# yxgeee/OpenIBL

Hardware: NVIDIA H100
Metric: images_per_sec_extraction (higher is better)
Workload: dtype f32 (bf16x3 split on wgmma, fp32 accumulate)

## Files before the change

include/iblb200.h:

```cpp
#ifndef IBLB200_H_
#define IBLB200_H_

#include <stddef.h>
#include <stdint.h>

#ifdef __cplusplus
extern "C" {
#endif

#define IBLB200_ABI_VERSION 1

typedef enum ibl_status {
  IBL_OK = 0,
  IBL_ERR_BAD_ARG = 1,
  IBL_ERR_NOT_READY = 2,
  IBL_ERR_CUDA = 3,
  IBL_ERR_NO_DEVICE = 4,
  IBL_ERR_OOM = 5,
  IBL_ERR_UNSUPPORTED = 6
} ibl_status;

typedef struct ibl_engine ibl_engine;

#define IBL_OUT_VLAD 0x1u
// ... 99 lines not shown
                   int m, int k_in, int k_out, float* out_dist, int64_t* out_idx, void* stream);
int ibl_l2dist_topk_host(ibl_engine* e, const float* q_host, int m, const float* db_host, int n,
                         int d, int k, float* out_dist_host, int64_t* out_idx_host, void* stream);

int ibl_knn_rowmax(ibl_engine* e, const float* X, int N, int d, int row0, int n_rows, int w, int64_t* out_idx,
                   float* out_dist, float* out_rowmax, void* stream);
int ibl_rerank_topk(ibl_engine* e, const float* X, int N, int m, int d, const int64_t* nbr_idx, const float* nbr_dist,
                    int w, const float* rowmax, int k1, int k2, float lambda_value, const int64_t* orig_idx, int k_orig,
                    int k, float* out_dist, int64_t* out_idx, void* stream);
int ibl_rerank_dense(ibl_engine* e, const float* qg, const float* qq, const float* gg, int m, int n, int k1, int k2,
                     double lambda_value, float* out_final, void* stream);

int ibl_gemm_nt(ibl_engine* e, const float* A, int m, const float* B, int n, int k, float alpha, float* C, int mode,
                void* stream);

int ibl_debug_dist_flagged(ibl_engine* e, int* count, void* stream);
int ibl_debug_dist_path(ibl_engine* e, int* path);
int ibl_debug_knn_flagged(ibl_engine* e, int* count, void* stream);
int ibl_debug_rerank_workspace_bytes(ibl_engine* e, uint64_t* bytes);
int ibl_selftest_tc(ibl_engine* e, float* max_rel_err);

int ibl_debug_conv3x3(ibl_engine* e, const float* x_nhwc, int N, int H, int W, int cin,
                      const float* w_oihw, const float* bias, int cout, int relu, int pool, int mode,
                      int bn_override, float* y_nhwc, void* stream);

int ibl_debug_gemm_tn(ibl_engine* e, const float* A, const float* B, float* C, void* stream);
int ibl_debug_umma_strided(ibl_engine* e, const void* A, int rows, const void* B, int s0, int group_rows,
                           int base_mode, float* D, void* stream);
int ibl_debug_umma_halo_view(ibl_engine* e, const void* A, int rows, const void* B, int s0, int group_rows,
                             int half_rows, float* D, void* stream);
int ibl_debug_conv1_fused(ibl_engine* e, const float* x, int N, int H, int W, void* y_hi, void* y_lo, void* stream);
int ibl_debug_time_layer(ibl_engine* e, int layer, const float* x, int N, int H, int W, int bn_override,
                         int reps, float* ms_out);

#ifdef __cplusplus
}
#endif
#endif
```

openibl_b200/_cabi.py:

```python
from __future__ import annotations

import ctypes
import os
from ctypes import POINTER, Structure, c_char, c_char_p, c_double, c_float, c_int, c_int64, c_size_t, c_uint, c_uint64, c_void_p

_HERE = os.path.dirname(os.path.abspath(__file__))
LIB_PATH = os.path.join(_HERE, "lib", "libiblb200.so")

IBL_OK = 0
STATUS_NAMES = {0: "IBL_OK", 1: "IBL_ERR_BAD_ARG", 2: "IBL_ERR_NOT_READY", 3: "IBL_ERR_CUDA",
                4: "IBL_ERR_NO_DEVICE", 5: "IBL_ERR_OOM", 6: "IBL_ERR_UNSUPPORTED"}
OUT_VLAD, OUT_PCA, OUT_POOL = 0x1, 0x2, 0x4
CONV_SIMT_FP32, CONV_TC_BF16X3 = 0, 1

_P = c_void_p


class JpegInfo(Structure):
    _fields_ = [("width", c_int), ("height", c_int), ("components", c_int), ("h_samp", c_int), ("v_samp", c_int),
                ("restart_interval", c_int), ("intervals", c_int), ("mcus", c_int), ("entropy_bytes", c_uint64),
                ("reason", c_char * 120)]


class ColorJitterParams(Structure):
# ... 27 lines not shown
    "ibl_l2_normalize_rows": (c_int, [_P, _P, c_int, c_int, _P, _P]),
    "ibl_extract": (c_int, [_P, _P, c_int, c_int, c_int, c_uint, _P, _P, _P]),
    "ibl_extract_host": (c_int, [_P, _P, c_int, c_int, c_int, c_uint, _P, _P, _P]),
    "ibl_extract_host_submit": (c_int, [_P, c_int, _P, c_int, c_int, c_int, c_uint, _P, _P, _P]),
    "ibl_extract_host_wait": (c_int, [_P, c_int]),
    "ibl_preprocess_u8": (c_int, [_P, _P, c_int, c_int, c_int, _P, _P, _P, _P]),
    "ibl_resize_bilinear_u8": (c_int, [_P, _P, c_int, c_int, c_int, c_int, c_int, _P, _P, c_int, _P, _P, c_int, _P, _P]),
    "ibl_extract_host_u8": (c_int, [_P, _P, c_int, c_int, c_int, _P, _P, c_uint, _P, _P, _P]),
    "ibl_jpeg_parse": (c_int, [c_char_p, c_size_t, POINTER(JpegInfo)]),
    "ibl_jpeg_decode_u8": (c_int, [_P, _P, _P, c_int, _P, _P, _P, _P, _P]),
    "ibl_color_jitter_u8": (c_int, [_P, _P, _P, _P, _P, POINTER(ColorJitterParams), c_int, _P]),
    "ibl_l2dist_dense": (c_int, [_P, _P, c_int, _P, c_int, c_int, _P, _P]),
    "ibl_l2dist_self": (c_int, [_P, _P, c_int, c_int, _P, _P]),
    "ibl_l2dist_topk": (c_int, [_P, _P, c_int, _P, c_int, c_int, c_int, c_int, c_int64, _P, _P, _P]),
    "ibl_topk_rows": (c_int, [_P, _P, c_int, c_int, c_int, _P, _P, _P]),
    "ibl_argsort_rows": (c_int, [_P, _P, c_int, c_int, _P, _P]),
    "ibl_topk_merge": (c_int, [_P, _P, _P, c_int, c_int, c_int, c_int, _P, _P, _P]),
    "ibl_l2dist_topk_host": (c_int, [_P, _P, c_int, _P, c_int, c_int, c_int, _P, _P, _P]),
    "ibl_knn_rowmax": (c_int, [_P, _P, c_int, c_int, c_int, c_int, c_int, _P, _P, _P, _P]),
    "ibl_rerank_topk": (c_int, [_P, _P, c_int, c_int, c_int, _P, _P, c_int, _P, c_int, c_int, c_float, _P, c_int,
                                c_int, _P, _P, _P]),
    "ibl_rerank_dense": (c_int, [_P, _P, _P, _P, c_int, c_int, c_int, c_int, c_double, _P, _P]),
    "ibl_debug_rerank_workspace_bytes": (c_int, [_P, POINTER(c_uint64)]),
    "ibl_debug_knn_flagged": (c_int, [_P, POINTER(c_int), _P]),
    "ibl_gemm_nt": (c_int, [_P, _P, c_int, _P, c_int, c_int, c_float, _P, c_int, _P]),
    "ibl_debug_dist_flagged": (c_int, [_P, POINTER(c_int), _P]),
    "ibl_debug_dist_path": (c_int, [_P, POINTER(c_int)]),
    "ibl_selftest_tc": (c_int, [_P, POINTER(c_float)]),
    "ibl_debug_gemm_tn": (c_int, [_P, _P, _P, _P, _P]),
    "ibl_debug_umma_strided": (c_int, [_P, _P, c_int, _P, c_int, c_int, c_int, _P, _P]),
    "ibl_debug_umma_halo_view": (c_int, [_P, _P, c_int, _P, c_int, c_int, c_int, _P, _P]),
    "ibl_debug_conv1_fused": (c_int, [_P, _P, c_int, c_int, c_int, _P, _P, _P]),
    "ibl_debug_time_layer": (c_int, [_P, c_int, _P, c_int, c_int, c_int, c_int, c_int, POINTER(c_float)]),
    "ibl_debug_conv3x3": (c_int, [_P, _P, c_int, c_int, c_int, c_int, _P, _P, c_int, c_int, c_int, c_int,
                                  c_int, _P, _P]),
}

_lib = None


class IblError(RuntimeError):
    def __init__(self, status: int, where: str, detail: str):
        self.status = status
        super().__init__(f"{where}: {STATUS_NAMES.get(status, status)}: {detail}")


def load(build_if_missing: bool = True) -> ctypes.CDLL:
    global _lib
    if _lib is not None:
        return _lib
    if not os.path.exists(LIB_PATH):
        if not build_if_missing:
            raise ImportError(f"{LIB_PATH} is missing; run `python -m openibl_b200.build`")
        from . import build as _build
        _build.build()
    lib = ctypes.CDLL(LIB_PATH)
    for name, (res, args) in SIGNATURES.items():
        fn = getattr(lib, name)
        fn.restype = res
        fn.argtypes = args
    _lib = lib
    return lib


def jpeg_parse(data: bytes) -> dict:
    lib = load()
# ... 15 lines not shown
```

openibl_b200/csrc/common.cuh:

```cuda
#pragma once
#include <cuda_runtime.h>
#include <cuda_bf16.h>
#include <stdint.h>
#include <stdio.h>
#include <atomic>
#include <string>

#include "../../include/iblb200.h"

namespace ibl {

void set_last_error(const std::string& s);

#define IBL_CUDA_OK(expr)                                                          \
  do {                                                                             \
    cudaError_t _e = (expr);                                                       \
    if (_e != cudaSuccess) {                                                       \
      ::ibl::set_last_error(std::string(#expr) + ": " + cudaGetErrorString(_e) +   \
                            " (" __FILE__ ":" + std::to_string(__LINE__) + ")");   \
      return IBL_ERR_CUDA;                                                         \
    }                                                                              \
  } while (0)

#define IBL_RET(expr)                 \
// ... 44 lines not shown
  int cin, cout;
  bool relu;
  bool pool;
};

struct ConvParams {
  float* w_tck = nullptr;
  float* bias = nullptr;
  __nv_bfloat16* w_hi = nullptr;
  __nv_bfloat16* w_lo = nullptr;
  int cin_pad = 0;
};

int launch_repack_weights(const float* w_oihw, int cout, int cin, ConvParams& p, cudaStream_t s);
int launch_conv3x3_simt(const float* x_nhwc, const ConvParams& p, int N, int H, int W, int cin,
                        int cout, bool relu, float* y_nhwc, cudaStream_t s);
int launch_conv1_1(const float* x_nchw, const ConvParams& p, int N, int H, int W, float* y_nhwc, cudaStream_t s);
int launch_maxpool2x2(const float* x, int N, int H, int W, int C, float* y, cudaStream_t s);
int launch_nhwc_to_nchw(const float* x, int N, int S, int C, float* y, cudaStream_t s);
int launch_u8_hwc_to_nchw_norm(const uint8_t* x, int N, int H, int W, const float* mean, const float* stdv, float* y,
                               cudaStream_t s);
int launch_global_maxpool_nhwc(const float* x, int N, int S, int C, float* y, cudaStream_t s);
int launch_planes_to_f32(const __nv_bfloat16* hi, const __nv_bfloat16* lo, size_t n, float* y,
                         cudaStream_t s);
int launch_f32_to_planes(const float* x, size_t n, __nv_bfloat16* hi, __nv_bfloat16* lo,
                         cudaStream_t s);

struct TcConvPlan;
int tc_driver_init();
int launch_conv3x3_tc(const __nv_bfloat16* x_hi, const __nv_bfloat16* x_lo, const ConvParams& p,
                      int N, int H, int W, int cin, int cout, bool relu, bool pool,
                      __nv_bfloat16* y_hi, __nv_bfloat16* y_lo, float* y_f32, cudaStream_t s,
                      float* ssq = nullptr, int* ssq_parts = nullptr);
int launch_conv1_fused_tc(const float* x_nchw, const float* w1_oihw, const float* bias1, const ConvParams& p2, int N, int H,
                          int W, __nv_bfloat16* y_hi, __nv_bfloat16* y_lo, cudaStream_t s);
int launch_maxpool2x2_planes(const __nv_bfloat16* hi, const __nv_bfloat16* lo, int N, int H, int W,
                             int C, __nv_bfloat16* yhi, __nv_bfloat16* ylo, cudaStream_t s);
int tc_selftest(float* max_rel_err, cudaStream_t s);
int launch_argsort_rows(const float* dist, long long ld, int m, int n, long long* idx, unsigned long long* scratch,
                        cudaStream_t s, uint64_t* launches);
int launch_resize_bilinear_u8(const uint8_t* x, int N, int Hin, int Win, int Hout, int Wout, const int* bounds_h,
                              const int* kk_h, int ksize_h, const int* bounds_v, const int* kk_v, int ksize_v,
                              uint8_t* tmp, uint8_t* out, cudaStream_t s, uint64_t* launches);
struct JpegWs;
void jpeg_ws_destroy(JpegWs* ws);
int jpeg_decode_u8(JpegWs** ws, const uint8_t* const* files, const size_t* lens, int N, uint8_t* out_u8,
                   const uint64_t* out_offsets, int* status, int* err_dev, cudaStream_t s, uint64_t* launches);
struct JitterWs;
void jitter_ws_destroy(JitterWs* ws);
int color_jitter_u8(JitterWs** ws, uint8_t* buf, const uint64_t* out_offsets, const int* H, const int* W,
                    const ibl_color_jitter_params* params, int N, cudaStream_t s, uint64_t* launches);
int launch_repack_weights_dgrad(const float* w_tck, int cout, int cin, __nv_bfloat16* w_hi, __nv_bfloat16* w_lo,
                                cudaStream_t s);
int launch_relu_mask_planes(const float* g, const float* y, size_t n, bool relu, __nv_bfloat16* hi, __nv_bfloat16* lo,
                            cudaStream_t s);
int launch_maxpool2x2_bwd(const float* x, const float* gy, int N, int H, int W, int C, float* gx, cudaStream_t s);
int wgrad_tc_splits(int N, int H, int W, int cin, int cout);
int launch_conv_wgrad_tc(const __nv_bfloat16* g_hi, const __nv_bfloat16* g_lo, const __nv_bfloat16* x_hi,
                         const __nv_bfloat16* x_lo, int N, int H, int W, int cin, int cout, float* part, int splits,
                         float* bpart, float* dw_oihw, float* db, cudaStream_t s);
int launch_conv1_1_wgrad(const float* x_nchw, const __nv_bfloat16* g_hi, const __nv_bfloat16* g_lo, int N, int H, int W,
                         float* part, float* dw_oihw, float* db, cudaStream_t s);
int launch_conv1_1_tc(const float* x_nchw, const float* w_oihw, const float* bias, int N, int H, int W,
                      __nv_bfloat16* y_hi, __nv_bfloat16* y_lo, cudaStream_t s);
int debug_gmma_strided(const void* A, int rows, const void* B, int s0, int group_rows, int half_rows, int base_mode,
                       float* D, cudaStream_t s);
// ... 88 lines not shown
```

openibl_b200/csrc/engine.cu:

```cuda
#include <stdlib.h>

#include <mutex>
#include <new>
#include <vector>

#include "common.cuh"

namespace ibl {

static thread_local std::string g_last_error;
void set_last_error(const std::string& s) { g_last_error = s; }
void tc_set_bn_override(int bn);

static const ConvLayer kVgg16[13] = {
    {3, 64, true, false},    {64, 64, true, true},
    {64, 128, true, false},  {128, 128, true, true},
    {128, 256, true, false}, {256, 256, true, false}, {256, 256, true, true},
    {256, 512, true, false}, {512, 512, true, false}, {512, 512, true, true},
    {512, 512, true, false}, {512, 512, true, false}, {512, 512, false, false}
};

struct DevBuf {
  void* p = nullptr;
  size_t cap = 0;
// ... 1241 lines not shown
  IBL_RET(e->act[1].ensure((in_e > out_e ? in_e : out_e) * 4));
  cudaEvent_t e0, e1;
  IBL_CUDA_OK(cudaEventCreate(&e0));
  IBL_CUDA_OK(cudaEventCreate(&e1));
  __nv_bfloat16* ih = e->act[0].as<__nv_bfloat16>();
  __nv_bfloat16* oh_ = e->act[1].as<__nv_bfloat16>();
  int rc = IBL_OK;
  if (layer > 0) rc = launch_f32_to_planes(x, in_e, ih, ih + in_e, nullptr);
  tc_set_bn_override(bn_override);
  for (int r = -1; r < reps && rc == IBL_OK; ++r) {
    if (r == 0) cudaEventRecord(e0, nullptr);
    if (fused1)
      rc = launch_conv1_fused_tc(x, e->w0_oihw, e->conv[0].bias, e->conv[1], N, H, W, oh_, oh_ + out_e, nullptr);
    else if (layer == 0)
      rc = launch_conv1_1_tc(x, e->w0_oihw, e->conv[0].bias, N, H, W, oh_, oh_ + out_e, nullptr);
    else
      rc = launch_conv3x3_tc(ih, ih + in_e, e->conv[layer], N, H, W, L.cin, L.cout, L.relu, L.pool,
                             layer == 12 ? nullptr : oh_, layer == 12 ? nullptr : oh_ + out_e,
                             layer == 12 ? e->act[1].as<float>() : nullptr, nullptr);
  }
  tc_set_bn_override(0);
  cudaEventRecord(e1, nullptr);
  cudaError_t ce = cudaEventSynchronize(e1);
  float ms = 0.f;
  cudaEventElapsedTime(&ms, e0, e1);
  cudaEventDestroy(e0);
  cudaEventDestroy(e1);
  if (rc == IBL_OK && ce != cudaSuccess) { set_last_error(cudaGetErrorString(ce)); return IBL_ERR_CUDA; }
  *ms_out = ms / reps;
  e->launches += reps + 1;
  return rc;
}

}
```

openibl_b200/csrc/tc_common.cuh:

```cuda
#pragma once
#include <cuda.h>
#include <cuda_runtime.h>
#include <stdint.h>

#include "wgmma.cuh"

namespace ibl {
namespace tc {

__device__ __forceinline__ uint32_t smem_u32(const void* p) {
  return static_cast<uint32_t>(__cvta_generic_to_shared(p));
}

__device__ __forceinline__ uint32_t warp_uniform(uint32_t v) { return __reduce_or_sync(0xffffffffu, v); }

__device__ __forceinline__ bool elect_one() {
  uint32_t pred;
  asm volatile(
      "{\n\t"
      ".reg .pred p;\n\t"
      "elect.sync _|p, 0xffffffff;\n\t"
      "selp.u32 %0, 1, 0, p;\n\t"
      "}"
      : "=r"(pred));
// ... 113 lines not shown
__device__ __forceinline__ void tma_load_2d_mc_a(uint32_t dst, const CUtensorMap* m, uint32_t bar_addr, int c0, int c1,
                                                 uint16_t mask) {
  asm volatile(
      "cp.async.bulk.tensor.2d.shared::cluster.global.mbarrier::complete_tx::bytes.multicast::cluster"
      " [%0], [%1, {%4, %5}], [%2], %3;" ::"r"(dst),
      "l"(reinterpret_cast<uint64_t>(m)), "r"(bar_addr), "h"(mask), "r"(c0), "r"(c1)
      : "memory");
}
__device__ __forceinline__ void tma_load_3d_mc_a(uint32_t dst, const CUtensorMap* m, uint32_t bar_addr, int c0, int c1,
                                                 int c2, uint16_t mask) {
  asm volatile(
      "cp.async.bulk.tensor.3d.shared::cluster.global.mbarrier::complete_tx::bytes.multicast::cluster"
      " [%0], [%1, {%4, %5, %6}], [%2], %3;" ::"r"(dst),
      "l"(reinterpret_cast<uint64_t>(m)), "r"(bar_addr), "h"(mask), "r"(c0), "r"(c1), "r"(c2)
      : "memory");
}
__device__ __forceinline__ void cluster_sync_all() {
  asm volatile("barrier.cluster.arrive.release.aligned;" ::: "memory");
  asm volatile("barrier.cluster.wait.acquire.aligned;" ::: "memory");
}
__device__ __forceinline__ uint32_t cluster_ctarank() {
  uint32_t r;
  asm volatile("mov.u32 %0, %%cluster_ctarank;" : "=r"(r));
  return r;
}
__device__ __forceinline__ uint32_t mapa_u32(uint32_t addr, uint32_t rank) {
  uint32_t r;
  asm volatile("mapa.shared::cluster.u32 %0, %1, %2;" : "=r"(r) : "r"(addr), "r"(rank));
  return r;
}
__device__ __forceinline__ void mbar_arrive_remote(uint32_t cluster_addr) {
  asm volatile("mbarrier.arrive.release.cluster.shared::cluster.b64 _, [%0];" ::"r"(cluster_addr) : "memory");
}

__device__ __forceinline__ void tma_prefetch_3d(const CUtensorMap* m, int c0, int c1, int c2) {
  asm volatile("cp.async.bulk.prefetch.tensor.3d.L2.global [%0, {%1, %2, %3}];" ::"l"(
                   reinterpret_cast<uint64_t>(m)),
               "r"(c0), "r"(c1), "r"(c2)
               : "memory");
}

__device__ __forceinline__ uint64_t gmma_desc_kmajor_sw128(uint32_t smem_addr) {
  uint64_t d = 0;
  d |= (uint64_t)((smem_addr >> 4) & 0x3fffu);
  d |= (uint64_t)1 << 16;
  d |= (uint64_t)(1024u >> 4) << 32;
  d |= (uint64_t)1 << 62;
  return d;
}
__device__ __forceinline__ uint64_t gmma_desc_kmajor_sw64(uint32_t smem_addr) {
  uint64_t d = 0;
  d |= (uint64_t)((smem_addr >> 4) & 0x3fffu);
  d |= (uint64_t)1 << 16;
  d |= (uint64_t)(512u >> 4) << 32;
  d |= (uint64_t)2 << 62;
  return d;
}
__device__ __forceinline__ uint64_t gmma_desc_mnmajor_sw128(uint32_t smem_addr, uint32_t lbo_bytes) {
  uint64_t d = 0;
  d |= (uint64_t)((smem_addr >> 4) & 0x3fffu);
  d |= (uint64_t)((lbo_bytes >> 4) & 0x3fffu) << 16;
  d |= (uint64_t)(1024u >> 4) << 32;
  d |= (uint64_t)1 << 62;
  return d;
}

// ... 65 lines not shown
```

openibl_b200/csrc/tc_conv.cu:

```cuda
#include "common.cuh"
#include "tc_common.cuh"

namespace ibl {

using namespace tc;

namespace tc {
EncodeTiledFn get_encode_tiled() {
  static const EncodeTiledFn fn = []() -> EncodeTiledFn {
    void* p = nullptr;
    cudaDriverEntryPointQueryResult qres;
    if (cudaGetDriverEntryPoint("cuTensorMapEncodeTiled", &p, cudaEnableDefault, &qres) ==
            cudaSuccess &&
        qres == cudaDriverEntryPointSuccess)
      return reinterpret_cast<EncodeTiledFn>(p);
    return nullptr;
  }();
  return fn;
}

int make_tmap(CUtensorMap* out, CUtensorMapDataType dt, int rank, const void* base,
              const uint64_t* dims, const uint64_t* strides_bytes, const uint32_t* box, int swizzle_bytes) {
  EncodeTiledFn enc = get_encode_tiled();
  if (!enc) {
    set_last_error("cuTensorMapEncodeTiled is not available (no CUDA driver?)");
    return IBL_ERR_NO_DEVICE;
  }
  cuuint64_t gdim[5];
  cuuint64_t gstr[5];
  cuuint32_t bx[5], es[5];
  for (int i = 0; i < rank; ++i) {
    gdim[i] = dims[i];
    bx[i] = box[i];
    es[i] = 1;
  }
  for (int i = 0; i + 1 < rank; ++i) gstr[i] = strides_bytes[i];
  CUresult r = enc(out, dt, (cuuint32_t)rank, const_cast<void*>(base), gdim, gstr, bx, es,
                   CU_TENSOR_MAP_INTERLEAVE_NONE,
                   swizzle_bytes == 64 ? CU_TENSOR_MAP_SWIZZLE_64B : CU_TENSOR_MAP_SWIZZLE_128B,
                   CU_TENSOR_MAP_L2_PROMOTION_L2_256B, CU_TENSOR_MAP_FLOAT_OOB_FILL_NONE);
  if (r != CUDA_SUCCESS) {
    set_last_error("cuTensorMapEncodeTiled failed with CUresult " + std::to_string((int)r));
    return IBL_ERR_CUDA;
  }
  return IBL_OK;
}
}

int tc_driver_init() { return get_encode_tiled() ? IBL_OK : IBL_ERR_NO_DEVICE; }

struct ConvTcArgs {
  int N, H, W, cin, cout;
  int tw_log2;
  int tiles_w, tiles_h;
  int n_tiles;
  int total_tiles;
  int relu, pool;
  const float* bias;
  __nv_bfloat16* y_hi;
  __nv_bfloat16* y_lo;
  float* y_f32;
  float* ssq;
  long long ssq_stride;
};

__device__ __forceinline__ uint32_t pack_bf16x2(float a, float b) {
  __nv_bfloat162 t = __floats2bfloat162_rn(a, b);
  return *reinterpret_cast<uint32_t*>(&t);
}

template <int BN>
__device__ __forceinline__ void conv_epilogue_tile(const ConvTcArgs& a, const Acc128<BN>& acc, float* stg, int img, int h0,
                                                   int w0, int n0, int nt, int r, int c, int dr_lanes, int bar = 1) {
  const int h = h0 + r, w = w0 + c;
  bool valid;
  long long pix;
  if (a.pool) {
    const int OH = a.H >> 1, OW = a.W >> 1;
    const int oh = h >> 1, ow = w >> 1;
    valid = oh < OH && ow < OW && img < a.N;
    pix = ((long long)img * OH + oh) * OW + ow;
  } else {
    valid = h < a.H && w < a.W && img < a.N;
    pix = ((long long)img * a.H + h) * a.W + w;
  }
  float ssq_acc = 0.f;
#pragma unroll
  for (int ch = 0; ch < BN / 32; ++ch) {
    uint32_t raw[32];
// ... 86 lines not shown
          ol4[j] = make_uint4(lo[4 * j], lo[4 * j + 1], lo[4 * j + 2], lo[4 * j + 3]);
        }
      }
    }
  }
  if (a.ssq && valid && !a.pool) a.ssq[(long long)nt * a.ssq_stride + pix] = ssq_acc;
}

constexpr int TC_BM = 128;
constexpr int TC_BK = 64;
constexpr int TC_A_BYTES = TC_BM * TC_BK * 2;

constexpr int TC_HALO_W = 10, TC_HALO_H = 18;
constexpr int TC_HALO_ROWS = TC_HALO_W * TC_HALO_H;
constexpr int TC_HALO_PLANE = 23 * 1024;
constexpr int TC_HALO_STAGE = 2 * TC_HALO_PLANE;

template <int BN, int STAGES, bool HALO = false, int NA = 0>
struct ConvTcSmem {
  static constexpr int THREADS = HALO ? 384 : 160;
  static constexpr int CONSUMERS = HALO ? 2 : 1;
  static constexpr int B_BYTES = BN * TC_BK * 2;
  static constexpr int STAGE_BYTES = HALO ? 2 * B_BYTES : 2 * TC_A_BYTES + 2 * B_BYTES;
  static constexpr int A_RING = HALO ? NA * TC_HALO_STAGE : 0;
  static constexpr int STG = CONSUMERS * ACC_STG_BYTES;
  static constexpr int BYTES = A_RING + STAGES * STAGE_BYTES + STG + 1024  + 256 ;
};

template <int BN, int STAGES, bool HALO, int NA>
__global__ void __launch_bounds__(ConvTcSmem<BN, STAGES, HALO, NA>::THREADS, 1)
conv3x3_tc_kernel(const __grid_constant__ CUtensorMap tm_xhi, const __grid_constant__ CUtensorMap tm_xlo,
                  const __grid_constant__ CUtensorMap tm_whi, const __grid_constant__ CUtensorMap tm_wlo,
                  const ConvTcArgs a) {
  extern __shared__ __align__(1024) uint8_t smem_raw[];
  uint8_t* smem = reinterpret_cast<uint8_t*>((reinterpret_cast<uintptr_t>(smem_raw) + 1023) & ~uintptr_t(1023));
  using L = ConvTcSmem<BN, STAGES, HALO, NA>;
  constexpr int B_BYTES = L::B_BYTES;
  constexpr int STAGE_BYTES = L::STAGE_BYTES;
  constexpr int A_RING = L::A_RING;
  uint8_t* ring = smem + A_RING;
  float* stg = reinterpret_cast<float*>(ring + STAGES * STAGE_BYTES);
  uint64_t* bars = reinterpret_cast<uint64_t*>(ring + STAGES * STAGE_BYTES + L::STG);
  uint64_t* full_bar = bars;
  uint64_t* empty_bar = bars + STAGES;
  uint64_t* afull_bar = bars + 2 * STAGES;
  uint64_t* aempty_bar = afull_bar + NA;
  uint64_t* order_bar = aempty_bar + NA;

  const int warp = threadIdx.x >> 5, lane = threadIdx.x & 31;
  const int worker = (int)blockIdx.x;
  const int n_workers = (int)gridDim.x;
  const int producer_warp = HALO ? 0 : 4;
  if (warp == producer_warp && lane == 0) {
    tma_prefetch_desc(&tm_xhi);
    tma_prefetch_desc(&tm_xlo);
    tma_prefetch_desc(&tm_whi);
    tma_prefetch_desc(&tm_wlo);
    for (int i = 0; i < STAGES; ++i) {
      mbar_init(&full_bar[i], 1);
      mbar_init(&empty_bar[i], 4);
    }
    for (int i = 0; i < NA; ++i) {
      mbar_init(&afull_bar[i], 1);
      mbar_init(&aempty_bar[i], 4);
    }
    if (HALO) {
      mbar_init(&order_bar[0], 4);
      mbar_init(&order_bar[1], 4);
    }
    fence_barrier_init();
    fence_proxy_async();
  }
  __syncthreads();

  const int TW = 1 << a.tw_log2;
  const int kchunks = a.cin / TC_BK;
  const int kiters = 9 * kchunks;
  const int tiles_per_img = a.tiles_h * a.tiles_w;
  auto coords = [&](int tile, int& img, int& h0, int& w0, int& nt) {
    nt = tile % a.n_tiles;
    const int pt = tile / a.n_tiles;
    img = pt / tiles_per_img;
    const int rem = pt - img * tiles_per_img;
    h0 = (rem / a.tiles_w) * (TC_BM >> a.tw_log2);
    w0 = (rem % a.tiles_w) * TW;
  };

  if (HALO && warp < 4) setmaxnreg_dec<40>();
  if (warp == producer_warp) {
    const uint32_t smem_a = warp_uniform(smem_u32(smem));
    const uint32_t ring_a = smem_a + A_RING;
    const uint32_t bars_a = ring_a + STAGES * STAGE_BYTES + L::STG;
    const uint32_t full_a = bars_a, empty_a = bars_a + 8 * STAGES;
    const uint32_t afull_a = bars_a + 16 * STAGES, aempty_a = afull_a + 8 * NA;
    auto load_w = [&](uint32_t st, uint32_t fb, int c0, int n0, int tap) {
      tma_load_3d_a(st, &tm_whi, fb, c0, n0, tap);
      tma_load_3d_a(st + B_BYTES, &tm_wlo, fb, c0, n0, tap);
    };
    int stage = 0;
    uint32_t phase = 0;
    if constexpr (HALO) {
      auto try_wait_warp = [&](uint32_t bar, uint32_t parity) -> bool {
        uint32_t ok = 0;
        if (lane == 0) {
          asm volatile(
              "{\n\t"
              ".reg .pred p;\n\t"
              "mbarrier.try_wait.parity.shared::cta.b64 p, [%1], %2;\n\t"
              "selp.u32 %0, 1, 0, p;\n\t"
              "}"
              : "=r"(ok)
              : "r"(bar), "r"(parity)
              : "memory");
        }
        return warp_uniform(ok) != 0;
      };
      int astage = 0;
      uint32_t aphase = 0;
      int tA = worker, kcA = 0, tB = worker, kcB = 0, tapB = 0;
      while (tB < a.total_tiles) {
        const uint32_t as_u = warp_uniform((uint32_t)astage);
        if (tA < a.total_tiles && try_wait_warp(aempty_a + 8 * as_u, aphase ^ 1)) {
          int img, h0, w0, nt;
          coords(tA, img, h0, w0, nt);
          img = (int)warp_uniform((uint32_t)img); h0 = (int)warp_uniform((uint32_t)h0);
          w0 = (int)warp_uniform((uint32_t)w0);
          const int c0 = (int)warp_uniform((uint32_t)(kcA * TC_BK));
          const uint32_t sa = smem_a + as_u * TC_HALO_STAGE;
          constexpr uint32_t kHaloBytes = 2u * TC_HALO_ROWS * 128u;
          if (elect_one()) {
            mbar_arrive_expect_tx_a(afull_a + 8 * as_u, kHaloBytes);
            tma_load_4d_a(sa, &tm_xhi, afull_a + 8 * as_u, c0, w0 - 1, h0 - 1, img);
            tma_load_4d_a(sa + TC_HALO_PLANE, &tm_xlo, afull_a + 8 * as_u, c0, w0 - 1, h0 - 1, img);
          }
          __syncwarp();
          if (++astage == NA) { astage = 0; aphase ^= 1; }
          if (++kcA == kchunks) { kcA = 0; tA += n_workers; }
          continue;
        }
        const uint32_t st_u = warp_uniform((uint32_t)stage);
        if (try_wait_warp(empty_a + 8 * st_u, phase ^ 1)) {
          int img, h0, w0, nt;
          coords(tB, img, h0, w0, nt);
          const int n0 = (int)warp_uniform((uint32_t)(nt * BN));
          const int c0 = (int)warp_uniform((uint32_t)(kcB * TC_BK));
          const int tap = (int)warp_uniform((uint32_t)tapB);
          const uint32_t st = ring_a + st_u * STAGE_BYTES;
          if (elect_one()) {
            mbar_arrive_expect_tx_a(full_a + 8 * st_u, STAGE_BYTES);
            load_w(st, full_a + 8 * st_u, c0, n0, tap);
          }
          __syncwarp();
          if (++stage == STAGES) { stage = 0; phase ^= 1; }
          if (++tapB == 9) { tapB = 0; if (++kcB == kchunks) { kcB = 0; tB += n_workers; } }
        }
      }
    } else
    for (int tile = worker; tile < a.total_tiles; tile += n_workers) {
      int img, h0, w0, nt;
      coords(tile, img, h0, w0, nt);
      img = (int)warp_uniform((uint32_t)img); h0 = (int)warp_uniform((uint32_t)h0);
      w0 = (int)warp_uniform((uint32_t)w0);
      const int n0 = (int)warp_uniform((uint32_t)(nt * BN));
      for (int kit = 0; kit < kiters; ++kit) {
        const int tap = (int)warp_uniform((uint32_t)(kit / kchunks));
        const int c0 = (int)warp_uniform((uint32_t)((kit - tap * kchunks) * TC_BK));
        const int kh = tap / 3 - 1, kw = tap % 3 - 1;
        const uint32_t st_u = warp_uniform((uint32_t)stage);
        mbar_wait_warp_a(empty_a + 8 * st_u, phase ^ 1);
        const uint32_t st = smem_a + st_u * STAGE_BYTES;
        if (elect_one()) {
          const uint32_t fb = full_a + 8 * st_u;
          mbar_arrive_expect_tx_a(fb, STAGE_BYTES);
          tma_load_4d_a(st, &tm_xhi, fb, c0, w0 + kw, h0 + kh, img);
          tma_load_4d_a(st + TC_A_BYTES, &tm_xlo, fb, c0, w0 + kw, h0 + kh, img);
          load_w(st + 2 * TC_A_BYTES, fb, c0, n0, tap);
        }
        __syncwarp();
        if (++stage == STAGES) { stage = 0; phase ^= 1; }
      }
    }
  } else if (!HALO || warp >= 4) {
    const uint32_t smem_a = smem_u32(smem);
    const uint32_t ring_a = smem_a + A_RING;
    auto release_w = [&](int st) {
      if (lane == 0) mbar_arrive(&empty_bar[st]);
    };
    if constexpr (HALO) {
    setmaxnreg_inc<232>();
    const int cw = warp / 4 - 1;
    const int bar = 1 + cw;
    float* my_stg = stg + cw * (ACC_STG_BYTES / 4);
    const int m = threadIdx.x & 127;
    const int r = TW == 16 ? (m >> 3) & 7 : m >> 3;
    const int c = TW == 16 ? ((m >> 6) << 3) | (m & 7) : m & 7;
    const uint32_t halo_w = (uint32_t)TW + 2;
    const uint64_t halo_desc = ((uint64_t)1 << 16) | ((uint64_t)((halo_w * 128) >> 4) << 32) | ((uint64_t)1 << 62);
    const uint64_t a_half = (TW == 16 ? 8u : 8u * halo_w) * 128u / 16u;
    for (int i = cw; worker + i * n_workers < a.total_tiles; i += 2) {
      int img, h0, w0, nt;
      coords(worker + i * n_workers, img, h0, w0, nt);
      int astage = (i * kchunks) % NA, stage = (i * kiters) % STAGES;
      uint32_t aphase = (uint32_t)((i * kchunks) / NA) & 1u, phase = (uint32_t)((i * kiters) / STAGES) & 1u;
      if (i > 0) mbar_wait(&order_bar[cw], (uint32_t)((i - 1) >> 1) & 1u);
      Acc128<BN> acc;
      int prev = -1, prev_a = -1;
      for (int kc = 0; kc < kchunks; ++kc) {
        mbar_wait(&afull_bar[astage], aphase);
        const uint32_t ha = smem_a + astage * TC_HALO_STAGE;
        for (int tap = 0; tap < 9; ++tap) {
          mbar_wait(&full_bar[stage], phase);
          const uint32_t toff = ((uint32_t)(tap / 3) * halo_w + (uint32_t)(tap % 3)) * 128u;
          const uint64_t a_hi = halo_desc | (uint64_t)(((ha + toff) >> 4) & 0x3fffu);
          const uint64_t a_lo = halo_desc | (uint64_t)(((ha + TC_HALO_PLANE + toff) >> 4) & 0x3fffu);
          const uint32_t sb = ring_a + stage * STAGE_BYTES;
          const uint64_t b_hi = gmma_desc_kmajor_sw128(sb), b_lo = gmma_desc_kmajor_sw128(sb + B_BYTES);
          wgmma_fence();
#pragma unroll
          for (int k = 0; k < TC_BK / 16; ++k) {
            const uint64_t ko = (uint64_t)(k * 2);
            acc.mma(a_lo + ko, a_lo + a_half + ko, b_hi + ko, (kc > 0 || tap > 0 || k > 0) ? 1u : 0u);
            acc.mma(a_hi + ko, a_hi + a_half + ko, b_lo + ko, 1u);
            acc.mma(a_hi + ko, a_hi + a_half + ko, b_hi + ko, 1u);
          }
          wgmma_commit();
          if (kc == kchunks - 1 && tap == 8 && lane == 0) mbar_arrive(&order_bar[cw ^ 1]);
          wgmma_wait<1>();
          if (prev >= 0) release_w(prev);
          if (prev_a >= 0) {
            if (lane == 0) mbar_arrive(&aempty_bar[prev_a]);
            prev_a = -1;
          }
          prev = stage;
          if (++stage == STAGES) { stage = 0; phase ^= 1; }
        }
        prev_a = astage;
        if (++astage == NA) { astage = 0; aphase ^= 1; }
      }
      wgmma_wait<0>();
      acc.fence_operands();
      release_w(prev);
      if (lane == 0) mbar_arrive(&aempty_bar[prev_a]);
      conv_epilogue_tile<BN>(a, acc, my_stg, img, h0, w0, nt * BN, nt, r, c, 8, bar);
    }
    } else {
    const int m = threadIdx.x;
    const int r = m >> a.tw_log2, c = m & (TW - 1);
    int stage = 0;
    uint32_t phase = 0;
    for (int tile = worker; tile < a.total_tiles; tile += n_workers) {
      int img, h0, w0, nt;
      coords(tile, img, h0, w0, nt);
      Acc128<BN> acc;
      int prev = -1;
      for (int kit = 0; kit < kiters; ++kit) {
        mbar_wait(&full_bar[stage], phase);
        const uint32_t sa = ring_a + stage * STAGE_BYTES;
        const uint64_t a_hi = gmma_desc_kmajor_sw128(sa), a_lo = gmma_desc_kmajor_sw128(sa + TC_A_BYTES);
        const uint64_t b_hi = gmma_desc_kmajor_sw128(sa + 2 * TC_A_BYTES);
        const uint64_t b_lo = gmma_desc_kmajor_sw128(sa + 2 * TC_A_BYTES + B_BYTES);
        constexpr uint64_t kHalf = (TC_BM / 2) * 128 / 16;
        wgmma_fence();
#pragma unroll
        for (int k = 0; k < TC_BK / 16; ++k) {
          const uint64_t ko = (uint64_t)(k * 2);
          acc.mma(a_lo + ko, a_lo + kHalf + ko, b_hi + ko, (kit > 0 || k > 0) ? 1u : 0u);
          acc.mma(a_hi + ko, a_hi + kHalf + ko, b_lo + ko, 1u);
          acc.mma(a_hi + ko, a_hi + kHalf + ko, b_hi + ko, 1u);
        }
        wgmma_commit();
        wgmma_wait<1>();
        if (prev >= 0) release_w(prev);
        prev = stage;
        if (++stage == STAGES) { stage = 0; phase ^= 1; }
      }
      wgmma_wait<0>();
      acc.fence_operands();
      if (prev >= 0) release_w(prev);
      conv_epilogue_tile<BN>(a, acc, stg, img, h0, w0, nt * BN, nt, r, c, TW);
    }
    }
  }
  __syncthreads();
}

template <int BN, int STAGES, bool HALO = false, int NA = 0>
static int launch_tc_variant(const CUtensorMap& xhi, const CUtensorMap& xlo, const CUtensorMap& whi,
                             const CUtensorMap& wlo, const ConvTcArgs& a, cudaStream_t s) {
  constexpr int smem = ConvTcSmem<BN, STAGES, HALO, NA>::BYTES;
  static_assert(smem <= 232448, "shared-memory budget");
  static DeviceOnce attr_done;
  if (!attr_done.done()) {
    IBL_CUDA_OK(cudaFuncSetAttribute(conv3x3_tc_kernel<BN, STAGES, HALO, NA>, cudaFuncAttributeMaxDynamicSharedMemorySize, smem));
    attr_done.mark();
  }
  const int sms = device_sm_count();
  const int grid = a.total_tiles < sms ? a.total_tiles : sms;
  conv3x3_tc_kernel<BN, STAGES, HALO, NA><<<grid, ConvTcSmem<BN, STAGES, HALO, NA>::THREADS, smem, s>>>(xhi, xlo, whi, wlo, a);
  IBL_CUDA_OK(cudaGetLastError());
  return IBL_OK;
}

static int g_tc_bn_override = 0;
void tc_set_bn_override(int bn) { g_tc_bn_override = bn; }

int launch_conv3x3_tc(const __nv_bfloat16* x_hi, const __nv_bfloat16* x_lo, const ConvParams& p,
                      int N, int H, int W, int cin, int cout, bool relu, bool pool,
                      __nv_bfloat16* y_hi, __nv_bfloat16* y_lo, float* y_f32, cudaStream_t s, float* ssq,
                      int* ssq_parts) {
  IBL_REQUIRE(cin % 64 == 0 && cout % 64 == 0, "tensor-core conv needs Cin%64==0 and Cout%64==0");
  IBL_REQUIRE(p.w_hi && p.w_lo, "tensor-core conv: weights were not re-laid-out");
  IBL_REQUIRE(H >= 1 && W >= 1 && N >= 1, "empty conv input");
  ConvTcArgs a{};
  a.N = N; a.H = H; a.W = W; a.cin = cin; a.cout = cout;
  auto waste = [&](int tw) {
    int th = 128 / tw;
    return (long long)cdiv(W, tw) * tw * cdiv(H, th) * th;
  };
  a.tw_log2 = (waste(16) <= waste(8)) ? 4 : 3;
  const int TW = 1 << a.tw_log2, TH = 128 / TW;
  a.tiles_w = cdiv(W, TW);
  a.tiles_h = cdiv(H, TH);
  int bn = cout % 128 == 0 ? 128 : 64;
  if (g_tc_bn_override && cout % g_tc_bn_override == 0 && (g_tc_bn_override == 64 || g_tc_bn_override == 128))
    bn = g_tc_bn_override;
  const bool halo = bn == 128;
  a.n_tiles = cout / bn;
  a.total_tiles = (int)((long long)N * a.tiles_h * a.tiles_w * a.n_tiles);
  a.relu = relu; a.pool = pool;
  a.bias = p.bias; a.y_hi = y_hi; a.y_lo = y_lo; a.y_f32 = y_f32;
  a.ssq = pool ? nullptr : ssq;
  a.ssq_stride = (long long)N * H * W;
  if (ssq_parts) *ssq_parts = a.n_tiles;

  CUtensorMap m_xhi, m_xlo, m_whi, m_wlo;
  {
    uint64_t dims[4] = {(uint64_t)cin, (uint64_t)W, (uint64_t)H, (uint64_t)N};
    uint64_t str[3] = {(uint64_t)cin * 2, (uint64_t)W * cin * 2, (uint64_t)H * W * cin * 2};
    uint32_t box[4] = {64, (uint32_t)(halo ? TW + 2 : TW), (uint32_t)(halo ? TH + 2 : TH), 1};
    IBL_RET(make_tmap(&m_xhi, CU_TENSOR_MAP_DATA_TYPE_BFLOAT16, 4, x_hi, dims, str, box));
    IBL_RET(make_tmap(&m_xlo, CU_TENSOR_MAP_DATA_TYPE_BFLOAT16, 4, x_lo, dims, str, box));
  }
  {
    uint64_t dims[3] = {(uint64_t)cin, (uint64_t)cout, 9};
    uint64_t str[2] = {(uint64_t)cin * 2, (uint64_t)cout * cin * 2};
    uint32_t box[3] = {64, (uint32_t)bn, 1};
    IBL_RET(make_tmap(&m_whi, CU_TENSOR_MAP_DATA_TYPE_BFLOAT16, 3, p.w_hi, dims, str, box));
    IBL_RET(make_tmap(&m_wlo, CU_TENSOR_MAP_DATA_TYPE_BFLOAT16, 3, p.w_lo, dims, str, box));
  }
  if (halo) return launch_tc_variant<128, 3, true, 2>(m_xhi, m_xlo, m_whi, m_wlo, a, s);
  return launch_tc_variant<64, 4>(m_xhi, m_xlo, m_whi, m_wlo, a, s);
}

struct Conv1FusedArgs {
  const float* x;
  const float* w1;
  const float* bias1;
  ConvTcArgs c2;
};

constexpr int F1_A1_ROWS = 192;
constexpr int F1_A1_PLANE = F1_A1_ROWS * 64;
constexpr int F1_W1_PLANE = 64 * 64;
constexpr int F1_W2_STAGE = 2 * 64 * TC_BK * 2;
constexpr int F1_W2_STAGES = 4;
constexpr int F1_OFF_W1 = 2 * TC_HALO_STAGE;
constexpr int F1_OFF_W2 = F1_OFF_W1 + 2 * F1_W1_PLANE;
constexpr int F1_OFF_STG = F1_OFF_W2 + F1_W2_STAGES * F1_W2_STAGE;
constexpr int F1_OFF_BAR = F1_OFF_STG + 2 * ACC_STG_BYTES;
constexpr int F1_SMEM = F1_OFF_BAR + 512 + 1024;
static_assert(2 * F1_A1_PLANE <= TC_HALO_STAGE, "A1 (hi | lo) is built inside the consumer's halo buffer");
static_assert(TC_HALO_STAGE % 1024 == 0 && F1_OFF_W1 % 512 == 0 && F1_OFF_W2 % 1024 == 0, "swizzle atom alignment");
static_assert(F1_SMEM <= 232448, "shared-memory budget of the fused conv1 kernel");

__device__ __forceinline__ void wgmma_n64_into_n128(float (&d)[64], uint64_t a, uint64_t b) {
  asm volatile(
      "{\n\t.reg .pred p;\n\tsetp.ne.b32 p, 1, 0;\n\t"
      "wgmma.mma_async.sync.aligned.m64n64k16.f32.bf16.bf16 {%0, %1, %2, %3, %4, %5, %6, %7, %8, %9, %10, %11, %12, %13, %14, %15, %16, %17, %18, %19, %20, %21, %22, %23, %24, %25, %26, %27, %28, %29, %30, %31}, %32, %33, p, 1, 1, 0, 0;\n\t}"
      : "+f"(d[0]), "+f"(d[1]), "+f"(d[2]), "+f"(d[3]), "+f"(d[4]), "+f"(d[5]), "+f"(d[6]), "+f"(d[7]), "+f"(d[8]), "+f"(d[9]), "+f"(d[10]), "+f"(d[11]), "+f"(d[12]), "+f"(d[13]), "+f"(d[14]), "+f"(d[15]), "+f"(d[16]), "+f"(d[17]), "+f"(d[18]), "+f"(d[19]), "+f"(d[20]), "+f"(d[21]), "+f"(d[22]), "+f"(d[23]), "+f"(d[24]), "+f"(d[25]), "+f"(d[26]), "+f"(d[27]), "+f"(d[28]), "+f"(d[29]), "+f"(d[30]), "+f"(d[31])
// ... 317 lines not shown
```

Before: 1203.

## Pair halo conv CTAs into 2-CTA clusters with multicast weight loads

Launches the BN=128 halo conv kernel as clusters of two CTAs that work on adjacent spatial tiles with the same output-channel tile. Each CTA loads half of the weight tile and multicasts it to both CTAs, so weight traffic per CTA is halved. Empty barriers now count consumers from both CTAs through remote arrives. An idle CTA in an odd tail still drains the weight pipeline so its partner can proceed. This adds cross-CTA synchronisation, and the CTAs of a cluster must progress in lockstep.

```diff
diff --git a/include/iblb200.h b/include/iblb200.h
--- a/include/iblb200.h
+++ b/include/iblb200.h
@@ -155,6 +155,7 @@
 int ibl_debug_conv1_fused(ibl_engine* e, const float* x, int N, int H, int W, void* y_hi, void* y_lo, void* stream);
 int ibl_debug_time_layer(ibl_engine* e, int layer, const float* x, int N, int H, int W, int bn_override,
                          int reps, float* ms_out);
+int ibl_debug_conv_clusters(ibl_engine* e, int* clusters);
 
 #ifdef __cplusplus
 }
diff --git a/openibl_b200/_cabi.py b/openibl_b200/_cabi.py
--- a/openibl_b200/_cabi.py
+++ b/openibl_b200/_cabi.py
@@ -83,6 +83,7 @@
     "ibl_debug_umma_halo_view": (c_int, [_P, _P, c_int, _P, c_int, c_int, c_int, _P, _P]),
     "ibl_debug_conv1_fused": (c_int, [_P, _P, c_int, c_int, c_int, _P, _P, _P]),
     "ibl_debug_time_layer": (c_int, [_P, c_int, _P, c_int, c_int, c_int, c_int, c_int, POINTER(c_float)]),
+    "ibl_debug_conv_clusters": (c_int, [_P, POINTER(c_int)]),
     "ibl_debug_conv3x3": (c_int, [_P, _P, c_int, c_int, c_int, c_int, _P, _P, c_int, c_int, c_int, c_int,
                                   c_int, _P, _P]),
 }
diff --git a/openibl_b200/csrc/common.cuh b/openibl_b200/csrc/common.cuh
--- a/openibl_b200/csrc/common.cuh
+++ b/openibl_b200/csrc/common.cuh
@@ -100,6 +100,7 @@
                       int N, int H, int W, int cin, int cout, bool relu, bool pool,
                       __nv_bfloat16* y_hi, __nv_bfloat16* y_lo, float* y_f32, cudaStream_t s,
                       float* ssq = nullptr, int* ssq_parts = nullptr);
+int conv3x3_tc_halo_clusters(int* clusters);
 int launch_conv1_fused_tc(const float* x_nchw, const float* w1_oihw, const float* bias1, const ConvParams& p2, int N, int H,
                           int W, __nv_bfloat16* y_hi, __nv_bfloat16* y_lo, cudaStream_t s);
 int launch_maxpool2x2_planes(const __nv_bfloat16* hi, const __nv_bfloat16* lo, int N, int H, int W,
diff --git a/openibl_b200/csrc/engine.cu b/openibl_b200/csrc/engine.cu
--- a/openibl_b200/csrc/engine.cu
+++ b/openibl_b200/csrc/engine.cu
@@ -1297,4 +1297,10 @@
   return rc;
 }
 
-}
+int ibl_debug_conv_clusters(ibl_engine* e, int* clusters) {
+  IBL_REQUIRE(e && clusters, "null argument");
+  DeviceGuard g(e->device);
+  return conv3x3_tc_halo_clusters(clusters);
+}
+
+}
diff --git a/openibl_b200/csrc/tc_common.cuh b/openibl_b200/csrc/tc_common.cuh
--- a/openibl_b200/csrc/tc_common.cuh
+++ b/openibl_b200/csrc/tc_common.cuh
@@ -169,6 +169,9 @@
 __device__ __forceinline__ void mbar_arrive_remote(uint32_t cluster_addr) {
   asm volatile("mbarrier.arrive.release.cluster.shared::cluster.b64 _, [%0];" ::"r"(cluster_addr) : "memory");
 }
+__device__ __forceinline__ void mbar_arrive_remote_cta(uint32_t cluster_addr) {
+  asm volatile("mbarrier.arrive.shared::cluster.b64 _, [%0];" ::"r"(cluster_addr) : "memory");
+}
 
 __device__ __forceinline__ void tma_prefetch_3d(const CUtensorMap* m, int c0, int c1, int c2) {
   asm volatile("cp.async.bulk.prefetch.tensor.3d.L2.global [%0, {%1, %2, %3}];" ::"l"(
diff --git a/openibl_b200/csrc/tc_conv.cu b/openibl_b200/csrc/tc_conv.cu
--- a/openibl_b200/csrc/tc_conv.cu
+++ b/openibl_b200/csrc/tc_conv.cu
@@ -55,6 +55,7 @@
   int tiles_w, tiles_h;
   int n_tiles;
   int total_tiles;
+  int units;
   int relu, pool;
   const float* bias;
   __nv_bfloat16* y_hi;
@@ -207,6 +208,8 @@
 conv3x3_tc_kernel(const __grid_constant__ CUtensorMap tm_xhi, const __grid_constant__ CUtensorMap tm_xlo,
                   const __grid_constant__ CUtensorMap tm_whi, const __grid_constant__ CUtensorMap tm_wlo,
                   const ConvTcArgs a) {
+  constexpr int CL = HALO ? 2 : 1;
+  auto cta_rank = [] { return HALO ? cluster_ctarank() : 0u; };
   extern __shared__ __align__(1024) uint8_t smem_raw[];
   uint8_t* smem = reinterpret_cast<uint8_t*>((reinterpret_cast<uintptr_t>(smem_raw) + 1023) & ~uintptr_t(1023));
   using L = ConvTcSmem<BN, STAGES, HALO, NA>;
@@ -223,8 +226,8 @@
   uint64_t* order_bar = aempty_bar + NA;
 
   const int warp = threadIdx.x >> 5, lane = threadIdx.x & 31;
-  const int worker = (int)blockIdx.x;
-  const int n_workers = (int)gridDim.x;
+  const int worker = (int)blockIdx.x / CL;
+  const int n_workers = (int)gridDim.x / CL;
   const int producer_warp = HALO ? 0 : 4;
   if (warp == producer_warp && lane == 0) {
     tma_prefetch_desc(&tm_xhi);
@@ -233,7 +236,7 @@
     tma_prefetch_desc(&tm_wlo);
     for (int i = 0; i < STAGES; ++i) {
       mbar_init(&full_bar[i], 1);
-      mbar_init(&empty_bar[i], 4);
+      mbar_init(&empty_bar[i], 4 * CL);
     }
     for (int i = 0; i < NA; ++i) {
       mbar_init(&afull_bar[i], 1);
@@ -247,14 +250,16 @@
     fence_proxy_async();
   }
   __syncthreads();
+  if (HALO) cluster_sync_all();
 
   const int TW = 1 << a.tw_log2;
   const int kchunks = a.cin / TC_BK;
   const int kiters = 9 * kchunks;
   const int tiles_per_img = a.tiles_h * a.tiles_w;
-  auto coords = [&](int tile, int& img, int& h0, int& w0, int& nt) {
-    nt = tile % a.n_tiles;
-    const int pt = tile / a.n_tiles;
+  auto live_units = [&] { return a.n_tiles * ((a.N * tiles_per_img + CL - 1 - (int)cta_rank()) / CL); };
+  auto coords = [&](int unit, int& img, int& h0, int& w0, int& nt) {
+    nt = unit % a.n_tiles;
+    const int pt = (unit / a.n_tiles) * CL + (int)cta_rank();
     img = pt / tiles_per_img;
     const int rem = pt - img * tiles_per_img;
     h0 = (rem / a.tiles_w) * (TC_BM >> a.tw_log2);
@@ -290,12 +295,15 @@
         }
         return warp_uniform(ok) != 0;
       };
+      const uint32_t rank_u = warp_uniform(cta_rank());
+      const int live_end = live_units();
+      const uint32_t w_half = rank_u * (B_BYTES / 2);
       int astage = 0;
       uint32_t aphase = 0;
       int tA = worker, kcA = 0, tB = worker, kcB = 0, tapB = 0;
-      while (tB < a.total_tiles) {
+      while (tB < a.units) {
         const uint32_t as_u = warp_uniform((uint32_t)astage);
-        if (tA < a.total_tiles && try_wait_warp(aempty_a + 8 * as_u, aphase ^ 1)) {
+        if (tA < live_end && try_wait_warp(aempty_a + 8 * as_u, aphase ^ 1)) {
           int img, h0, w0, nt;
           coords(tA, img, h0, w0, nt);
           img = (int)warp_uniform((uint32_t)img); h0 = (int)warp_uniform((uint32_t)h0);
@@ -315,15 +323,14 @@
         }
         const uint32_t st_u = warp_uniform((uint32_t)stage);
         if (try_wait_warp(empty_a + 8 * st_u, phase ^ 1)) {
-          int img, h0, w0, nt;
-          coords(tB, img, h0, w0, nt);
-          const int n0 = (int)warp_uniform((uint32_t)(nt * BN));
+          const int n0 = (int)warp_uniform((uint32_t)((tB % a.n_tiles) * BN + (int)rank_u * (BN / 2)));
           const int c0 = (int)warp_uniform((uint32_t)(kcB * TC_BK));
           const int tap = (int)warp_uniform((uint32_t)tapB);
-          const uint32_t st = ring_a + st_u * STAGE_BYTES;
+          const uint32_t st = ring_a + st_u * STAGE_BYTES + w_half, fb = full_a + 8 * st_u;
           if (elect_one()) {
-            mbar_arrive_expect_tx_a(full_a + 8 * st_u, STAGE_BYTES);
-            load_w(st, full_a + 8 * st_u, c0, n0, tap);
+            mbar_arrive_expect_tx_a(fb, STAGE_BYTES);
+            tma_load_3d_mc_a(st, &tm_whi, fb, c0, n0, tap, 0x3);
+            tma_load_3d_mc_a(st + B_BYTES, &tm_wlo, fb, c0, n0, tap, 0x3);
           }
           __syncwarp();
           if (++stage == STAGES) { stage = 0; phase ^= 1; }
@@ -331,7 +338,7 @@
         }
       }
     } else
-    for (int tile = worker; tile < a.total_tiles; tile += n_workers) {
+    for (int tile = worker; tile < a.units; tile += n_workers) {
       int img, h0, w0, nt;
       coords(tile, img, h0, w0, nt);
       img = (int)warp_uniform((uint32_t)img); h0 = (int)warp_uniform((uint32_t)h0);
@@ -359,7 +366,10 @@
     const uint32_t smem_a = smem_u32(smem);
     const uint32_t ring_a = smem_a + A_RING;
     auto release_w = [&](int st) {
-      if (lane == 0) mbar_arrive(&empty_bar[st]);
+      if (lane == 0) {
+        mbar_arrive(&empty_bar[st]);
+        if (HALO) mbar_arrive_remote_cta(mapa_u32(smem_u32(&empty_bar[st]), cluster_ctarank() ^ 1u));
+      }
     };
     if constexpr (HALO) {
     setmaxnreg_inc<232>();
@@ -372,12 +382,23 @@
     const uint32_t halo_w = (uint32_t)TW + 2;
     const uint64_t halo_desc = ((uint64_t)1 << 16) | ((uint64_t)((halo_w * 128) >> 4) << 32) | ((uint64_t)1 << 62);
     const uint64_t a_half = (TW == 16 ? 8u : 8u * halo_w) * 128u / 16u;
-    for (int i = cw; worker + i * n_workers < a.total_tiles; i += 2) {
+    auto unit_of = [&](int i) { return (int)(blockIdx.x / CL + i * (gridDim.x / CL)); };
+    for (int i = cw; unit_of(i) < a.units; i += 2) {
+      const int unit = unit_of(i);
       int img, h0, w0, nt;
-      coords(worker + i * n_workers, img, h0, w0, nt);
+      coords(unit, img, h0, w0, nt);
       int astage = (i * kchunks) % NA, stage = (i * kiters) % STAGES;
       uint32_t aphase = (uint32_t)((i * kchunks) / NA) & 1u, phase = (uint32_t)((i * kiters) / STAGES) & 1u;
       if (i > 0) mbar_wait(&order_bar[cw], (uint32_t)((i - 1) >> 1) & 1u);
+      if (unit >= live_units()) {
+        for (int k = 0; k < kiters; ++k) {
+          mbar_wait(&full_bar[stage], phase);
+          if (k == kiters - 1 && lane == 0) mbar_arrive(&order_bar[cw ^ 1]);
+          release_w(stage);
+          if (++stage == STAGES) { stage = 0; phase ^= 1; }
+        }
+        continue;
+      }
       Acc128<BN> acc;
       int prev = -1, prev_a = -1;
       for (int kc = 0; kc < kchunks; ++kc) {
@@ -423,7 +444,7 @@
     const int r = m >> a.tw_log2, c = m & (TW - 1);
     int stage = 0;
     uint32_t phase = 0;
-    for (int tile = worker; tile < a.total_tiles; tile += n_workers) {
+    for (int tile = worker; tile < a.units; tile += n_workers) {
       int img, h0, w0, nt;
       coords(tile, img, h0, w0, nt);
       Acc128<BN> acc;
@@ -457,24 +478,62 @@
     }
   }
   __syncthreads();
+  if (HALO) cluster_sync_all();
+}
+
+template <int BN, int STAGES, bool HALO, int NA>
+static cudaLaunchConfig_t tc_variant_config(int grid, cudaStream_t s, cudaLaunchAttribute* attr) {
+  cudaLaunchConfig_t cfg{};
+  cfg.gridDim = dim3(grid);
+  cfg.blockDim = dim3(ConvTcSmem<BN, STAGES, HALO, NA>::THREADS);
+  cfg.dynamicSmemBytes = ConvTcSmem<BN, STAGES, HALO, NA>::BYTES;
+  cfg.stream = s;
+  if (HALO) {
+    attr[0].id = cudaLaunchAttributeClusterDimension;
+    attr[0].val.clusterDim.x = 2;
+    attr[0].val.clusterDim.y = 1;
+    attr[0].val.clusterDim.z = 1;
+    cfg.attrs = attr;
+    cfg.numAttrs = 1;
+  }
+  return cfg;
+}
+
+template <int BN, int STAGES, bool HALO, int NA>
+static int tc_variant_workers(int* workers) {
+  constexpr int smem = ConvTcSmem<BN, STAGES, HALO, NA>::BYTES;
+  static_assert(smem <= 232448, "shared-memory budget");
+  static DeviceOnce attr_done;
+  static std::atomic<int> clusters[256];
+  if (!attr_done.done()) {
+    IBL_CUDA_OK(cudaFuncSetAttribute(conv3x3_tc_kernel<BN, STAGES, HALO, NA>, cudaFuncAttributeMaxDynamicSharedMemorySize, smem));
+    if (HALO) {
+      cudaLaunchAttribute attr[1];
+      const cudaLaunchConfig_t cfg = tc_variant_config<BN, STAGES, HALO, NA>(2, nullptr, attr);
+      int n = 0;
+      IBL_CUDA_OK(cudaOccupancyMaxActiveClusters(&n, conv3x3_tc_kernel<BN, STAGES, HALO, NA>, &cfg));
+      IBL_REQUIRE(n >= 1, "the halo conv kernel's clusters of two CTAs do not fit on this device");
+      clusters[DeviceOnce::cur()].store(n);
+    }
+    attr_done.mark();
+  }
+  *workers = HALO ? clusters[DeviceOnce::cur()].load() : device_sm_count();
+  return IBL_OK;
 }
 
 template <int BN, int STAGES, bool HALO = false, int NA = 0>
 static int launch_tc_variant(const CUtensorMap& xhi, const CUtensorMap& xlo, const CUtensorMap& whi,
                              const CUtensorMap& wlo, const ConvTcArgs& a, cudaStream_t s) {
-  constexpr int smem = ConvTcSmem<BN, STAGES, HALO, NA>::BYTES;
-  static_assert(smem <= 232448, "shared-memory budget");
-  static DeviceOnce attr_done;
-  if (!attr_done.done()) {
-    IBL_CUDA_OK(cudaFuncSetAttribute(conv3x3_tc_kernel<BN, STAGES, HALO, NA>, cudaFuncAttributeMaxDynamicSharedMemorySize, smem));
-    attr_done.mark();
-  }
-  const int sms = device_sm_count();
-  const int grid = a.total_tiles < sms ? a.total_tiles : sms;
-  conv3x3_tc_kernel<BN, STAGES, HALO, NA><<<grid, ConvTcSmem<BN, STAGES, HALO, NA>::THREADS, smem, s>>>(xhi, xlo, whi, wlo, a);
-  IBL_CUDA_OK(cudaGetLastError());
+  int workers = 0;
+  IBL_RET((tc_variant_workers<BN, STAGES, HALO, NA>(&workers)));
+  const int grid = (HALO ? 2 : 1) * (a.units < workers ? a.units : workers);
+  cudaLaunchAttribute attr[1];
+  const cudaLaunchConfig_t cfg = tc_variant_config<BN, STAGES, HALO, NA>(grid, s, attr);
+  IBL_CUDA_OK(cudaLaunchKernelEx(&cfg, conv3x3_tc_kernel<BN, STAGES, HALO, NA>, xhi, xlo, whi, wlo, a));
   return IBL_OK;
 }
+
+int conv3x3_tc_halo_clusters(int* clusters) { return tc_variant_workers<128, 3, true, 2>(clusters); }
 
 static int g_tc_bn_override = 0;
 void tc_set_bn_override(int bn) { g_tc_bn_override = bn; }
@@ -502,6 +561,7 @@
   const bool halo = bn == 128;
   a.n_tiles = cout / bn;
   a.total_tiles = (int)((long long)N * a.tiles_h * a.tiles_w * a.n_tiles);
+  a.units = halo ? (int)(((long long)N * a.tiles_h * a.tiles_w + 1) / 2 * a.n_tiles) : a.total_tiles;
   a.relu = relu; a.pool = pool;
   a.bias = p.bias; a.y_hi = y_hi; a.y_lo = y_lo; a.y_f32 = y_f32;
   a.ssq = pool ? nullptr : ssq;
@@ -519,7 +579,7 @@
   {
     uint64_t dims[3] = {(uint64_t)cin, (uint64_t)cout, 9};
     uint64_t str[2] = {(uint64_t)cin * 2, (uint64_t)cout * cin * 2};
-    uint32_t box[3] = {64, (uint32_t)bn, 1};
+    uint32_t box[3] = {64, (uint32_t)(halo ? bn / 2 : bn), 1};
     IBL_RET(make_tmap(&m_whi, CU_TENSOR_MAP_DATA_TYPE_BFLOAT16, 3, p.w_hi, dims, str, box));
     IBL_RET(make_tmap(&m_wlo, CU_TENSOR_MAP_DATA_TYPE_BFLOAT16, 3, p.w_lo, dims, str, box));
   }
```

Result: faster. 1219, median of 6 (+1.3%).
